# kimkyeonghun/MSA

Hardware: AMD Instinct MI355X
Metric: train-step samples/sec (higher is better)
Workload: dtype bf16; 1 GPU; MMBertForPretraining train step, 3 passes S=50/550/550, 12-layer d=768 heads=12 vocab=30522, T=50 A=500 V=500, dropout on, AdamW; per_gpu_batch=16, global_batch=16, parallelism=dp1, scores_dtype=bf16, mlm_backward=labelled rows only (exact: unlabelled rows have zero CE gradient), deterministic=True

## Files before the change

### msa_amd/csrc/gemm.hip

```cpp
#include "common.h"
#include <atomic>
#include <cstdio>
#include <cstdlib>
#include <cstring>
#include <type_traits>

typedef __attribute__((ext_vector_type(4))) unsigned u32x4;
typedef __attribute__((ext_vector_type(2))) unsigned u32x2;

#define EPI_BIAS 1
#define EPI_GELU 2
#define EPI_RESID 4
#define EPI_GELU_BWD 8
#define EPI_OUT_F32 16

struct GemmNT {
    const bf16_t* A; const bf16_t* B; void* C;
    const float* bias; const bf16_t* R; bf16_t* aux; const bf16_t* U; const float* alpha_dev;
    int M, N, K, lda, ldb, ldc, ldr, ldaux, ldu;
    float alpha;
    uint32_t drop_stream, drop_thr16; float drop_scale;
    int kt_per_split; long long split_stride;
    int* tile_counter; int* tile_counter_next;
    int queue_xcd;
    int group_m;
};

__device__ __forceinline__ int xcd_remap(int bid, int nwg) {
    const int q = nwg >> 3, r = nwg & 7, x = bid & 7, j = bid >> 3;
    return (x < r ? x * (q + 1) : r * (q + 1) + (x - r) * q) + j;
}

__device__ __forceinline__ void ntp_tile_mn(int t, int tiles_m, int tiles_n, int gm, int& tm, int& tn) {
    if (gm <= 1) { tm = t / tiles_n; tn = t - tm * tiles_n; return; }
    const int per = gm * tiles_n, g = t / per, r = t - g * per;
    const int gs = min(gm, tiles_m - g * gm);
    tn = r / gs;
    tm = g * gm + (r - tn * gs);
}

template <int EPI>
__device__ __forceinline__ void epi_store(const GemmNT& p, int m, int n, float (&v)[4]) {
    if constexpr (EPI & EPI_BIAS) {
        const float4 b = *(const float4*)(p.bias + n);
        v[0] += b.x; v[1] += b.y; v[2] += b.z; v[3] += b.w;
    }
    if constexpr (EPI & EPI_GELU) {
        if (p.aux) {
            bf16x4 u = {f2bf(v[0]), f2bf(v[1]), f2bf(v[2]), f2bf(v[3])};
            *(bf16x4*)(p.aux + (size_t)m * p.ldaux + n) = u;
        }
#pragma unroll
        for (int r = 0; r < 4; ++r) v[r] = gelu_erf(v[r]);
    }
    if constexpr (EPI & EPI_GELU_BWD) {
        const bf16x4 u = *(const bf16x4*)(p.U + (size_t)m * p.ldu + n);
#pragma unroll
        for (int r = 0; r < 4; ++r) v[r] *= gelu_erf_grad(bf2f(u[r]));
    }
    if constexpr (EPI & EPI_RESID) {
        if (p.drop_thr16) {
            bool k[4];
            mmb_keep4(p.drop_stream, (uint64_t)m * p.N + n, p.drop_thr16, k);
#pragma unroll
            for (int r = 0; r < 4; ++r) v[r] = k[r] ? v[r] * p.drop_scale : 0.f;
        }
        const bf16x4 rr = *(const bf16x4*)(p.R + (size_t)m * p.ldr + n);
#pragma unroll
        for (int r = 0; r < 4; ++r) v[r] += bf2f(rr[r]);
    }
    if constexpr (EPI & EPI_OUT_F32) {
        *(float4*)((float*)p.C + (size_t)m * p.ldc + n) = make_float4(v[0], v[1], v[2], v[3]);
    } else {
        bf16x4 o = {f2bf(v[0]), f2bf(v[1]), f2bf(v[2]), f2bf(v[3])};
        *(bf16x4*)((bf16_t*)p.C + (size_t)m * p.ldc + n) = o;
    }
}

template <int EPI>
__device__ __forceinline__ void epi_store8(const GemmNT& p, int m, int n, float (&v)[8]) {
    if constexpr (EPI & EPI_BIAS) {
        const float4 b0 = *(const float4*)(p.bias + n), b1 = *(const float4*)(p.bias + n + 4);
        v[0] += b0.x; v[1] += b0.y; v[2] += b0.z; v[3] += b0.w; v[4] += b1.x; v[5] += b1.y; v[6] += b1.z; v[7] += b1.w;
    }
    if constexpr (EPI & EPI_GELU) {
        if (p.aux) {
            bf16x8 u;
#pragma unroll
            for (int r = 0; r < 8; ++r) u[r] = f2bf(v[r]);
            *(bf16x8*)(p.aux + (size_t)m * p.ldaux + n) = u;
        }
#pragma unroll
        for (int r = 0; r < 8; ++r) v[r] = gelu_erf(v[r]);
    }
    if constexpr (EPI & EPI_GELU_BWD) {
        const bf16x8 u = *(const bf16x8*)(p.U + (size_t)m * p.ldu + n);
#pragma unroll
        for (int r = 0; r < 8; ++r) v[r] *= gelu_erf_grad(bf2f(u[r]));
    }
    if constexpr (EPI & EPI_RESID) {
        if (p.drop_thr16) {
            bool k0[4], k1[4];
            const uint64_t idx = (uint64_t)m * p.N + n;
            mmb_keep4(p.drop_stream, idx, p.drop_thr16, k0);
            mmb_keep4(p.drop_stream, idx + 4, p.drop_thr16, k1);
#pragma unroll
            for (int r = 0; r < 4; ++r) { v[r] = k0[r] ? v[r] * p.drop_scale : 0.f; v[4 + r] = k1[r] ? v[4 + r] * p.drop_scale : 0.f; }
        }
        const bf16x8 rr = *(const bf16x8*)(p.R + (size_t)m * p.ldr + n);
#pragma unroll
        for (int r = 0; r < 8; ++r) v[r] += bf2f(rr[r]);
    }
    if constexpr (EPI & EPI_OUT_F32) {
        float* c = (float*)p.C + (size_t)m * p.ldc + n;
        *(float4*)c = make_float4(v[0], v[1], v[2], v[3]);
        *(float4*)(c + 4) = make_float4(v[4], v[5], v[6], v[7]);
    } else {
        bf16x8 o;
#pragma unroll
        for (int r = 0; r < 8; ++r) o[r] = f2bf(v[r]);
        *(bf16x8*)((bf16_t*)p.C + (size_t)m * p.ldc + n) = o;
    }
}

template <int EPI>
__global__ __launch_bounds__(256, 2) void gemm_nt_kernel(const GemmNT p) {
    extern __shared__ __attribute__((aligned(16))) char smem[];
    const int tid = threadIdx.x, lane = tid & 63;
    const int wave = __builtin_amdgcn_readfirstlane(tid >> 6);
    const int wm = wave >> 1, wn = wave & 1;
    const int tiles_n = (p.N + 127) >> 7, tiles_m = (p.M + 127) >> 7;
    const int tile = xcd_remap(blockIdx.x, tiles_m * tiles_n);
    const int m0 = (tile / tiles_n) << 7, n0 = (tile % tiles_n) << 7;
    const int kt0 = p.kt_per_split ? (int)blockIdx.z * p.kt_per_split : 0;
    const int kt1 = p.kt_per_split ? min(p.K >> 6, kt0 + p.kt_per_split) : (p.K >> 6);

    const int srow = lane >> 3, schunk = (lane & 7) ^ srow;
    const bf16_t* a_src[4]; const bf16_t* b_src[4];
#pragma unroll
    for (int i = 0; i < 4; ++i) {
        const int r = (wave * 4 + i) * 8 + srow;
        const int ra = min(m0 + r, p.M - 1), rb = min(n0 + r, p.N - 1);
        a_src[i] = p.A + (size_t)ra * p.lda + schunk * 8;
        b_src[i] = p.B + (size_t)rb * p.ldb + schunk * 8;
    }
    auto stage = [&](int buf, int kt) {
        char* base = smem + buf * 32768 + wave * 4096;
#pragma unroll
        for (int i = 0; i < 4; ++i) {
            __builtin_amdgcn_global_load_lds(GPTR(a_src[i] + kt * 64), LPTR(base + i * 1024), 16, 0, 0);
            __builtin_amdgcn_global_load_lds(GPTR(b_src[i] + kt * 64), LPTR(base + 16384 + i * 1024), 16, 0, 0);
        }
    };

    f32x4 acc[4][4];
#pragma unroll
    for (int i = 0; i < 4; ++i)
#pragma unroll
        for (int j = 0; j < 4; ++j) acc[i][j] = (f32x4){0.f, 0.f, 0.f, 0.f};

    const int fr = lane & 15, fq = lane >> 4;
    auto compute = [&](int buf) {
        const char* As = smem + buf * 32768;
        const char* Bs = As + 16384;
#pragma unroll
        for (int kk = 0; kk < 2; ++kk) {
            bf16x8 af[4], bfr[4];
#pragma unroll
            for (int i = 0; i < 4; ++i) {
                const int ra = wm * 64 + i * 16 + fr, rb = wn * 64 + i * 16 + fr;
                af[i] = *(const bf16x8*)(As + ra * 128 + (((kk * 4 + fq) ^ (ra & 7)) << 4));
                bfr[i] = *(const bf16x8*)(Bs + rb * 128 + (((kk * 4 + fq) ^ (rb & 7)) << 4));
            }
#pragma unroll
            for (int i = 0; i < 4; ++i)
#pragma unroll
                for (int j = 0; j < 4; ++j)
                    acc[i][j] = __builtin_amdgcn_mfma_f32_16x16x32_bf16(bfr[j], af[i], acc[i][j], 0, 0, 0);
        }
    };

    stage(0, kt0);
    asm volatile("s_waitcnt vmcnt(0)" ::: "memory");
    __syncthreads();
    int cur = 0;
    for (int kt = kt0; kt < kt1 - 1; ++kt) {
        stage(cur ^ 1, kt + 1);
        compute(cur);
        asm volatile("s_waitcnt vmcnt(0)" ::: "memory");
        __syncthreads();
        cur ^= 1;
    }
    compute(cur);

    const float alpha = p.alpha * (p.alpha_dev ? *p.alpha_dev : 1.0f);
#pragma unroll
    for (int i = 0; i < 4; ++i) {
        const int m = m0 + wm * 64 + i * 16 + fr;
        if (m >= p.M) continue;
#pragma unroll
        for (int j = 0; j < 4; ++j) {
            const int n = n0 + wn * 64 + j * 16 + fq * 4;
            if (n >= p.N) continue;
            float v[4];
#pragma unroll
            for (int r = 0; r < 4; ++r) v[r] = acc[i][j][r] * alpha;
            if constexpr (EPI == EPI_OUT_F32) {
                if (p.kt_per_split) {
                    *(float4*)((float*)p.C + (size_t)blockIdx.z * p.split_stride + (size_t)m * p.ldc + n) = make_float4(v[0], v[1], v[2], v[3]);
                    continue;
                }
            }
            epi_store<EPI>(p, m, n, v);
        }
    }
}

template <int EPI>
static int launch_nt(hipStream_t s, const GemmNT& p) {
    const int tiles = ((p.M + 127) / 128) * ((p.N + 127) / 128);
    static std::atomic<unsigned long long> attr_done{0};
    if (int e = mmb_allow_lds((const void*)gemm_nt_kernel<EPI>, 65536, attr_done)) return e;
    hipLaunchKernelGGL(gemm_nt_kernel<EPI>, dim3(tiles), dim3(256), 65536, s, p);
    MMB_CHECK_LAUNCH();
    return 0;
}

#ifdef MMB_STAMPS
__device__ unsigned long long* g_stamps = nullptr;
#define MMB_STAMP(var) { __builtin_amdgcn_sched_barrier(0); asm volatile("s_memtime %0\n\ts_waitcnt lgkmcnt(0)" : "=s"(var) :: "memory"); __builtin_amdgcn_sched_barrier(0); }
#else
#define MMB_STAMP(var)
#endif

static std::atomic<int> g_nt_force{0};
static int device_cus() { return mmb_device_cus(); }

__host__ __device__ constexpr int mmb_waitcnt(int vm, int lgkm) { return (vm & 15) | ((vm >> 4) << 14) | 0x70 | (lgkm << 8); }

template <int OFF>
__device__ __forceinline__ void lds_read16f(f32x4& dst, uint32_t lds_addr) {
    asm volatile("ds_read_b128 %0, %1 offset:%2" : "=v"(dst) : "v"(lds_addr), "i"(OFF) : "memory");
}


template <int EPI, bool MULTI, int MQ>
__global__ __launch_bounds__(512, 2) void gemm_nt8_kernel(const GemmNT p) {
#if __HIP_DEVICE_COMPILE__
    extern __shared__ __attribute__((aligned(16))) char smem[];
    const int tid = threadIdx.x, lane = tid & 63;
    const int wave = __builtin_amdgcn_readfirstlane(tid >> 6);
    const int wr = wave >> 2, wc = wave & 3;
    constexpr int MQ0 = (MQ == 7) ? 4 : MQ, MQ1 = (MQ == 7) ? 3 : MQ, NB = MQ0 + MQ1;
    constexpr int BMT = 32 * NB;
    const int tiles_n = (p.N + 255) >> 8, tiles_m = (p.M + BMT - 1) / BMT;
    const int ntiles = tiles_m * tiles_n, G = gridDim.x;
    const int nt = p.K >> 6;
    const float alpha_all = __builtin_bit_cast(float, __builtin_amdgcn_readfirstlane(__builtin_bit_cast(int, p.alpha * (p.alpha_dev ? *p.alpha_dev : 1.0f))));

    const auto rsA = __builtin_amdgcn_make_buffer_rsrc((void*)p.A, 0, (int)((uint32_t)p.M * (uint32_t)p.lda * 2u), 0x00020000);
    const auto rsB = __builtin_amdgcn_make_buffer_rsrc((void*)p.B, 0, (int)((uint32_t)p.N * (uint32_t)p.ldb * 2u), 0x00020000);
    struct Src { uint32_t a[2][2], b[2][2]; };
    auto set_src = [&](int v, Src& o) {
        int l = lane;
        asm volatile("" : "+v"(l));
        int tmi, tni;
        ntp_tile_mn(xcd_remap(v, ntiles), tiles_m, tiles_n, p.group_m, tmi, tni);
        const int tm0 = tmi * BMT, tn0 = tni << 8;
        const int pos = l & 7;
#pragma unroll
        for (int i = 0; i < 2; ++i) {
            const int j = wave + 8 * i, r = 8 * j + (l >> 3);
            const uint32_t chunk_a = (uint32_t)(pos ^ ((r >> 1) & 7));
            const uint32_t chunk_b = (uint32_t)(pos ^ (((r >> 1) & 1) | (((r >> 3) & 3) << 1)));
#pragma unroll
            for (int h = 0; h < 2; ++h) {
                const int mqh = h ? MQ1 : MQ0;
                const int ga = tm0 + (r / (16 * mqh)) * (16 * NB) + (h ? 16 * MQ0 : 0) + (r % (16 * mqh));
                const int gb = tn0 + (r >> 5) * 64 + h * 32 + (r & 31);
                o.a[h][i] = ((uint32_t)min(ga, p.M - 1) * (uint32_t)p.lda + chunk_a * 8u) * 2u;
                o.b[h][i] = ((uint32_t)min(gb, p.N - 1) * (uint32_t)p.ldb + chunk_b * 8u) * 2u;
            }
        }
    };
    Src cur;
    set_src(blockIdx.x, cur);
    Src nxt_store;
    Src& nxt = MULTI ? nxt_store : cur;
    if constexpr (MULTI) nxt_store = cur;
    auto stage_c = [&](auto apw_c, int buf, int which, const Src& o, int kt) {
        constexpr int APW = decltype(apw_c)::value;
        const uint32_t kb = (uint32_t)kt * 128u;
        const int h = which >> 1;
        char* base = smem + buf * 65536 + ((which & 1) ? 0 : 32768) + h * 16384 + wave * 1024;
        if (which & 1) {
            __builtin_amdgcn_raw_ptr_buffer_load_lds(rsA, LPTR(base), 16, o.a[h][0], kb, 0, 0);
            const int mqh = h ? MQ1 : MQ0;
            if (mqh == 4 || (mqh == 3 && APW == 2)) __builtin_amdgcn_raw_ptr_buffer_load_lds(rsA, LPTR(base + 8192), 16, o.a[h][1], kb, 0, 0);
        } else {
            __builtin_amdgcn_raw_ptr_buffer_load_lds(rsB, LPTR(base), 16, o.b[h][0], kb, 0, 0);
            __builtin_amdgcn_raw_ptr_buffer_load_lds(rsB, LPTR(base + 8192), 16, o.b[h][1], kb, 0, 0);
        }
    };

    typedef const __attribute__((address_space(3))) char* lds_cptr;
    typedef const __attribute__((address_space(3))) bf16x8* lds_frag;
    const int fr = lane & 15, fq = lane >> 4;
    const int swa = ((fq ^ (fr >> 1)) & 7) << 4;
    const int swb = ((fq ^ (((fr >> 1) & 1) | ((fr >> 2) << 1))) & 7) << 4;
    const lds_cptr a_rd = (lds_cptr)LPTR(smem) + (wr * (16 * MQ0) + fr) * 128;
    const lds_cptr b_rd = (lds_cptr)LPTR(smem) + 32768 + (wc * 32 + 8 * (fr >> 2) + (fr & 3)) * 128;
    lds_cptr a_rd1 = a_rd + 65536, b_rd1 = b_rd + 65536;
    asm volatile("" : "+v"(a_rd1), "+v"(b_rd1));

    bf16x8 af[2][MQ0], b0f[2][2], b1f[2][2];
    f32x4 acc[NB][4];

    auto read_a = [&](int buf, int h) {
        lds_cptr ab = buf ? a_rd1 : a_rd;
        if (MQ0 != MQ1 && h) ab += wr * (16 * (MQ1 - MQ0) * 128);
#pragma unroll
        for (int ks = 0; ks < 2; ++ks)
#pragma unroll
            for (int i = 0; i < MQ0; ++i)
                if (i < (h ? MQ1 : MQ0)) af[ks][i] = *(lds_frag)(ab + h * 16384 + i * 2048 + (swa ^ (ks * 64)));
    };
    auto read_b = [&](int buf, int h, bf16x8 (&bf)[2][2]) {
        const lds_cptr bb = buf ? b_rd1 : b_rd;
#pragma unroll
        for (int ks = 0; ks < 2; ++ks)
#pragma unroll
            for (int j = 0; j < 2; ++j) bf[ks][j] = *(lds_frag)(bb + h * 16384 + j * 512 + (swb ^ (ks * 64)));
    };
    auto mma = [&](int qa, int qb, const bf16x8 (&bf)[2][2], bool first) {
#pragma unroll
        for (int ks = 0; ks < 2; ++ks)
#pragma unroll
            for (int i = 0; i < MQ0; ++i)
#pragma unroll
                for (int j = 0; j < 2; ++j) {
                    if (i >= (qa ? MQ1 : MQ0)) continue;
                    f32x4& c = acc[qa * MQ0 + i][qb * 2 + j];
                    c = __builtin_amdgcn_mfma_f32_16x16x32_bf16(bf[ks][j], af[ks][i], (first && ks == 0) ? (f32x4){0.f, 0.f, 0.f, 0.f} : c, 0, 0, 0);
                }
    };

    auto body = [&](auto apw_c) {
    constexpr int INFL = 4 + (MQ0 == 4 ? 2 : (MQ0 == 2 ? 1 : decltype(apw_c)::value));
    auto stage = [&](int buf, int which, const Src& o, int kt) { stage_c(apw_c, buf, which, o, kt); };
    const int qx = (MULTI && p.queue_xcd) ? (int)(blockIdx.x & 7) : 0, qs = (MULTI && p.queue_xcd) ? 8 : 1;
    auto queue_fetch = [](int* counter) {
        int r;
        asm volatile("s_nop 4\n\tglobal_atomic_add %0, %1, %2, %3 sc0" : "=&v"(r) : "v"(0), "v"(1), "s"(counter) : "memory");
        return r;
    };
    auto vq_write = [&](int value) {
        const uint32_t vq_addr = (uint32_t)(size_t)LPTR(smem) + 131072u;
        asm volatile("ds_write_b32 %0, %1\n\ts_waitcnt lgkmcnt(0)" :: "v"(vq_addr), "v"(value) : "memory");
    };
    int first_fetch = 0;
    if constexpr (MULTI) { if (p.tile_counter && tid == 0) first_fetch = queue_fetch(p.tile_counter + qx); }
    stage(0, 0, cur, 0); stage(0, 1, cur, 0); stage(0, 2, cur, 0); stage(0, 3, cur, 0);
    stage(1, 0, cur, 1); stage(1, 1, cur, 1); stage(1, 2, cur, 1);
    __builtin_amdgcn_s_waitcnt(mmb_waitcnt(INFL, 15));
    if constexpr (MULTI) {
        if (p.tile_counter && tid == 0) {
            asm volatile("" : "+v"(first_fetch) :: "memory");
            vq_write(G + qs * first_fetch + qx);
        }
    }
    __builtin_amdgcn_s_barrier();
    if (wr == 1) __builtin_amdgcn_s_barrier();

#define NT8_PHASE(READS, LGK_BEFORE_BARRIER, STAGE, VMWAIT, QA, QB, BF, FIRST)                                       \
    {                                                                                                               \
        READS;                                                                                                      \
        STAGE;                                                                                                      \
        if (LGK_BEFORE_BARRIER >= 0) __builtin_amdgcn_s_waitcnt(mmb_waitcnt(63, LGK_BEFORE_BARRIER < 0 ? 0 : LGK_BEFORE_BARRIER)); \
        if (VMWAIT >= 0) __builtin_amdgcn_s_waitcnt(mmb_waitcnt(VMWAIT < 0 ? 0 : VMWAIT, 15));                       \
        __builtin_amdgcn_s_barrier();                                                                               \
        __builtin_amdgcn_s_waitcnt(mmb_waitcnt(63, 0));                                                             \
        __builtin_amdgcn_sched_barrier(0);                                                                          \
        __builtin_amdgcn_s_setprio(1);                                                                              \
        mma(QA, QB, BF, FIRST);                                                                                     \
        __builtin_amdgcn_s_setprio(0);                                                                              \
        __builtin_amdgcn_s_barrier();                                                                               \
        __builtin_amdgcn_sched_barrier(0);                                                                          \
    }
#define NT8_KTILE(D, S1, K1, S2, K2, FIRST)                                                                                   \
    NT8_PHASE((read_b(D, 0, b0f), __builtin_amdgcn_sched_barrier(0), read_a(D, 0)), 2 * MQ0, stage(D ^ 1, 3, S1, K1), -1, 0, 0, b0f, FIRST) \
    NT8_PHASE(read_b(D, 1, b1f), -1, stage(D, 0, S2, K2), -1, 0, 1, b1f, FIRST)                                               \
    NT8_PHASE(read_a(D, 1), -1, stage(D, 1, S2, K2), -1, 1, 1, b1f, FIRST)                                                    \
    NT8_PHASE((void)0, -1, stage(D, 2, S2, K2), INFL, 1, 0, b0f, FIRST)

    for (int v = blockIdx.x, vn = ntiles; v < ntiles; v = vn) {
        int tmi, tni;
// ... 495 lines not shown
                if (accum) { v.x += old[u][jb].x; v.y += old[u][jb].y; v.z += old[u][jb].z; v.w += old[u][jb].w; }
                *(float4*)(out + (size_t)n * K + k) = v;
            }
        }
    }
    if (do_bias) {
        float* red = (float*)smem;
        float v[2][2];
#pragma unroll
        for (int hb = 0; hb < 2; ++hb)
#pragma unroll
            for (int j = 0; j < 2; ++j) {
                float s = bsum[hb][j];
                s += __shfl_xor(s, 16, 64);
                s += __shfl_xor(s, 32, 64);
                v[hb][j] = s;
            }
        __syncthreads();
        if (wr == 1 && fq == 0) {
#pragma unroll
            for (int hb = 0; hb < 2; ++hb)
#pragma unroll
                for (int j = 0; j < 2; ++j) red[((wc * 2 + hb) * 2 + j) * 16 + fr] = v[hb][j];
        }
        __syncthreads();
        if (wr == 0 && fq == 0) {
#pragma unroll
            for (int hb = 0; hb < 2; ++hb)
#pragma unroll
                for (int j = 0; j < 2; ++j) {
                    const int n = n0 + hb * 128 + wc * 32 + j * 16 + fr;
                    if (n >= N) continue;
                    const float bv = (v[hb][j] + red[((wc * 2 + hb) * 2 + j) * 16 + fr]) * alpha;
                    if (split > 0 && gq.bias_slab) gq.bias_slab[(size_t)(split - 1) * gq.bias_stride + bias_off + n] = bv;
                    else atomicAdd(biasp + n, bv);
                }
        }
    }
#ifdef MMB_STAMPS
    if (g_stamps && tid == 0) {
        asm volatile("s_waitcnt vmcnt(0)" ::: "memory");
        asm volatile("s_memrealtime %0\n\ts_waitcnt lgkmcnt(0)" : "=s"(tr1) :: "memory");
        unsigned long long te;
        MMB_STAMP(te)
        unsigned long long* o = g_stamps + ((size_t)(blockIdx.y * gridDim.x + blockIdx.x)) * 6;
        o[0] = ts1 - ts0; o[1] = (unsigned long long)(nt > 0 ? 2 * nt : 0); o[2] = te - ts1; o[3] = 1; o[4] = tr0; o[5] = tr1;
    }
#endif
#endif
}

struct TNReduce { float* W[TN_MAXP]; long long off[TN_MAXP + 1]; int nprob, splits, accumulate; long long slab_stride;
                  float* bias[TN_MAXP]; long long boff[TN_MAXP + 1]; const float* bias_slab; long long bias_stride; };
__global__ void tn_reduce_kernel(const TNReduce r, const float* __restrict__ slab) {
    if (r.bias_slab) {
        const long long nb = r.boff[r.nprob];
        for (long long e = blockIdx.x * (long long)blockDim.x + threadIdx.x; e < nb; e += (long long)gridDim.x * blockDim.x) {
            int lo = 0, hi = r.nprob - 1;
            while (lo < hi) { const int mid = (lo + hi + 1) >> 1; if (r.boff[mid] <= e) lo = mid; else hi = mid - 1; }
            if (!r.bias[lo]) continue;
            float v = r.bias[lo][e - r.boff[lo]];
            for (int s = 0; s + 1 < r.splits; ++s) v += r.bias_slab[(size_t)s * r.bias_stride + e];
            r.bias[lo][e - r.boff[lo]] = v;
        }
    }
    const long long total4 = r.off[r.nprob] >> 2;
    for (long long i = blockIdx.x * (long long)blockDim.x + threadIdx.x; i < total4; i += (long long)gridDim.x * blockDim.x) {
        const long long e = i << 2;
        int lo = 0, hi = r.nprob - 1;
        while (lo < hi) { const int mid = (lo + hi + 1) >> 1; if (r.off[mid] <= e) lo = mid; else hi = mid - 1; }
        float* W = r.W[lo];
        const long long o = r.off[lo];
        float4* dst = (float4*)(W + (e - o));
        float4 v = *dst;
        for (int s = 0; s + 1 < r.splits; ++s) {
            const float4 t = *(const float4*)(slab + (size_t)s * r.slab_stride + e);
            v.x += t.x; v.y += t.y; v.z += t.z; v.w += t.w;
        }
        *dst = v;
    }
}

__global__ __launch_bounds__(256) void colsum_kernel(const bf16_t* __restrict__ X, int M, int N, int ldx, float* __restrict__ out, float alpha, const float* alpha_dev, int rows_per_block) {
    const int lane = threadIdx.x & 63, sub = threadIdx.x >> 6;
    const int n = (blockIdx.x * 64 + lane) * 8;
    const int mbeg = blockIdx.y * rows_per_block, mend = min(M, mbeg + rows_per_block);
    float s[8];
#pragma unroll
    for (int r = 0; r < 8; ++r) s[r] = 0.f;
    if (n < N) {
        int m = mbeg + sub;
        for (; m + 12 < mend; m += 16) {
            bf16x8 v[4];
#pragma unroll
            for (int u = 0; u < 4; ++u) v[u] = *(const bf16x8*)(X + (size_t)(m + 4 * u) * ldx + n);
#pragma unroll
            for (int u = 0; u < 4; ++u)
#pragma unroll
                for (int r = 0; r < 8; ++r) s[r] += bf2f(v[u][r]);
        }
        for (; m < mend; m += 4) {
            const bf16x8 v = *(const bf16x8*)(X + (size_t)m * ldx + n);
#pragma unroll
            for (int r = 0; r < 8; ++r) s[r] += bf2f(v[r]);
        }
    }
    __shared__ float red[4][64][9];
#pragma unroll
    for (int r = 0; r < 8; ++r) red[sub][lane][r] = s[r];
    __syncthreads();
    if (sub == 0 && n < N) {
        const float a = alpha * (alpha_dev ? *alpha_dev : 1.0f);
#pragma unroll
        for (int r = 0; r < 8; ++r)
            atomicAdd(out + n + r, (red[0][lane][r] + red[1][lane][r] + red[2][lane][r] + red[3][lane][r]) * a);
    }
}

extern "C" {

__global__ void nt_splitk_reduce_kernel(const float* __restrict__ slabs, int splits, long long stride, int M, int N, bf16_t* __restrict__ C, int ldc,
                                        const bf16_t* __restrict__ R, int ldr) {
    const long long i = ((long long)blockIdx.x * blockDim.x + threadIdx.x) * 4;
    if (i >= (long long)M * N) return;
    float4 a = *(const float4*)(slabs + i);
    for (int z = 1; z < splits; ++z) { const float4 b = *(const float4*)(slabs + z * stride + i); a.x += b.x; a.y += b.y; a.z += b.z; a.w += b.w; }
    const int m = (int)(i / N), n = (int)(i - (long long)m * N);
    if (R) { const bf16x4 r = *(const bf16x4*)(R + (size_t)m * ldr + n); a.x += bf2f(r[0]); a.y += bf2f(r[1]); a.z += bf2f(r[2]); a.w += bf2f(r[3]); }
    bf16x4 o = {f2bf(a.x), f2bf(a.y), f2bf(a.z), f2bf(a.w)};
    *(bf16x4*)(C + (size_t)m * ldc + n) = o;
}

static int nt_splitk_plan(int M, int N, int K) {
    const int tiles = ((M + 127) / 128) * ((N + 127) / 128), kt = K >> 6;
    int splits = (2 * device_cus() + tiles - 1) / tiles;
    if (splits > kt / 4) splits = kt / 4;
    if (splits < 1) splits = 1;
    return splits;
}
size_t mmbert_gemm_nt_splitk_workspace(int M, int N, int K) { return (size_t)nt_splitk_plan(M, N, K) * M * N * sizeof(float); }

int mmbert_gemm_nt_splitk(hipStream_t stream, const void* A, int lda, const void* B, int ldb, void* C, int ldc,
                          int M, int N, int K, void* workspace, const void* R, int ldr) {
    if (M <= 0 || N <= 0) return 0;
    if (K <= 0 || (K & 63) || (N & 3) || (lda & 7) || (ldb & 7) || (ldc & 3) || !workspace || (R && (ldr & 3))) return -1;
    GemmNT p = {};
    p.A = (const bf16_t*)A; p.B = (const bf16_t*)B; p.C = workspace; p.M = M; p.N = N; p.K = K; p.lda = lda; p.ldb = ldb; p.ldc = N;
    p.alpha = 1.0f;
    const int splits = nt_splitk_plan(M, N, K), kt = K >> 6;
    p.kt_per_split = (kt + splits - 1) / splits;
    p.split_stride = (long long)M * N;
    const int zs = (kt + p.kt_per_split - 1) / p.kt_per_split;
    static std::atomic<unsigned long long> attr_done{0};
    if (int e = mmb_allow_lds((const void*)gemm_nt_kernel<EPI_OUT_F32>, 65536, attr_done)) return e;
    hipLaunchKernelGGL(gemm_nt_kernel<EPI_OUT_F32>, dim3(((M + 127) / 128) * ((N + 127) / 128), 1, zs), dim3(256), 65536, stream, p);
    MMB_CHECK_LAUNCH();
    const long long n4 = ((long long)M * N + 3) / 4;
    hipLaunchKernelGGL(nt_splitk_reduce_kernel, dim3((unsigned)((n4 + 255) / 256)), dim3(256), 0, stream, (const float*)workspace, zs, p.split_stride, M, N, (bf16_t*)C, ldc,
                       (const bf16_t*)R, ldr);
    MMB_CHECK_LAUNCH();
    return 0;
}

int mmbert_gemm_nt(hipStream_t stream, const void* A, int lda, const void* B, int ldb, void* C, int ldc,
                   int M, int N, int K, int epi, const float* bias, const void* R, int ldr, void* aux, int ldaux,
                   const void* U, int ldu, float alpha, const float* alpha_dev,
                   uint32_t drop_stream, uint32_t drop_thr16, float drop_scale, int* tile_queue) {
    if (M <= 0 || N <= 0) return 0;
    if (K <= 0 || (K & 63) || (N & 3) || (lda & 7) || (ldb & 7) || (ldc & 3)) return -1;
    GemmNT p;
    p.A = (const bf16_t*)A; p.B = (const bf16_t*)B; p.C = C; p.bias = bias; p.R = (const bf16_t*)R;
    p.aux = (bf16_t*)aux; p.U = (const bf16_t*)U; p.alpha_dev = alpha_dev;
    p.M = M; p.N = N; p.K = K; p.lda = lda; p.ldb = ldb; p.ldc = ldc; p.ldr = ldr; p.ldaux = ldaux; p.ldu = ldu;
    p.alpha = alpha; p.drop_stream = drop_stream; p.drop_thr16 = drop_thr16; p.drop_scale = drop_scale;
    p.kt_per_split = 0; p.split_stride = 0; p.group_m = 1;
    p.tile_counter = tile_queue; p.tile_counter_next = tile_queue ? tile_queue + 8 : nullptr;
    switch (epi) {
        case 0: return dispatch_nt<0>(stream, p);
        case EPI_BIAS: return dispatch_nt<EPI_BIAS>(stream, p);
        case EPI_BIAS | EPI_GELU: return dispatch_nt<EPI_BIAS | EPI_GELU>(stream, p);
        case EPI_BIAS | EPI_RESID: return dispatch_nt<EPI_BIAS | EPI_RESID>(stream, p);
        case EPI_RESID: return dispatch_nt<EPI_RESID>(stream, p);
        case EPI_GELU_BWD: return dispatch_nt<EPI_GELU_BWD>(stream, p);
        case EPI_OUT_F32: return dispatch_nt<EPI_OUT_F32>(stream, p);
        case EPI_BIAS | EPI_OUT_F32: return dispatch_nt<EPI_BIAS | EPI_OUT_F32>(stream, p);
        default: return -2;
    }
}

int mmbert_gemm_nt_describe(int M, int N, int K, int epi, int with_queue, int* out) {
    if (!out || M <= 0 || N <= 0 || K <= 0) return -1;
    GemmNT p = {};
    p.M = M; p.N = N; p.K = K; p.lda = K; p.ldb = K; p.ldc = N; p.ldr = (epi & (EPI_RESID)) ? N : 0; p.ldaux = (epi & EPI_GELU) ? N : 0;
    p.ldu = (epi & EPI_GELU_BWD) ? N : 0;
    static int dummy_queue[16];
    p.tile_counter = with_queue ? dummy_queue : nullptr;
    const NTChoice c = nt_choose(p, epi);
    const int cus = device_cus();
    out[0] = c.kernel; out[1] = c.bm; out[2] = c.kernel == NTK_128 ? 128 : 256; out[3] = c.tiles; out[4] = c.workgroups;
    out[5] = (int)(100.0 * c.tiles / cus + 0.5); out[6] = c.group_m; out[7] = cus;
    return 0;
}

#ifdef MMB_STAMPS
int mmbert_debug_set_stamps(void* buf) {
    return (int)hipMemcpyToSymbol(HIP_SYMBOL(g_stamps), &buf, sizeof(buf));
}
#endif
void mmbert_gemm_nt_force(int mode) {
    g_nt_force.store((mode == 1 || mode == 8 || mode == 128 || mode == 192 || mode == 224 || mode == 256) ? mode : 0);
}

static std::atomic<int> g_tn_splits{0};
void mmbert_gemm_tn_force_splits(int splits) { g_tn_splits.store(splits); }
static std::atomic<int> g_tn_one_launch{0};
void mmbert_gemm_tn_force_one_launch(int on) { g_tn_one_launch.store(on ? 1 : 0); }
static int tn_plan(int nprob, const int* N, const int* K, int M, int* splits_out, int* tiles_out) {
    int tiles = 0;
    double elems = 0;
    for (int i = 0; i < nprob; ++i) { tiles += ((N[i] + 255) / 256) * ((K[i] + 255) / 256); elems += (double)N[i] * K[i]; }
    constexpr double T_ROW = 21e-9, T_FIX = 8e-6;
    const int slots = device_cus();
    const int max_splits = (M + 511) / 512;
    double cost[9];
    double best_cost = 1e300;
    int top = 1;
    for (int sp = 1; sp <= 8 && sp <= (max_splits < 1 ? 1 : max_splits); ++sp) {
        const long long wgs = (long long)tiles * sp;
        const long long rounds = (wgs + slots - 1) / slots;
        const double rows = (double)((M + sp - 1) / sp);
        cost[sp] = (rows * T_ROW + T_FIX) * (double)rounds + (sp - 1) * elems * 8.0 / 9.4e12;
        if (cost[sp] < best_cost) best_cost = cost[sp];
        top = sp;
    }
    int best = 1;
    for (int sp = 1; sp <= top; ++sp)
        if (cost[sp] <= 1.03 * best_cost) { best = sp; break; }
    int splits = best;
    if (tiles >= slots && nprob > 8) splits = 1;
    if (g_tn_splits.load() > 0) splits = g_tn_splits.load();
    if (splits > max_splits) splits = max_splits;
    if (splits < 1) splits = 1;
    *splits_out = splits; *tiles_out = tiles;
    return 0;
}

size_t mmbert_gemm_tn_grouped_workspace(int nprob, const int* N, const int* K, int M, int* splits_out) {
    int splits, tiles;
    tn_plan(nprob, N, K, M, &splits, &tiles);
    if (splits_out) *splits_out = splits;
    if (splits == 1) return 0;
    size_t elems = 0, cols = 0;
    for (int i = 0; i < nprob; ++i) { elems += (size_t)N[i] * K[i]; cols += (size_t)N[i]; }
    return (size_t)(splits - 1) * (elems + cols) * sizeof(float);
}

size_t mmbert_gemm_tn_workspace(int M, int N, int K, int* splits_out) {
    return mmbert_gemm_tn_grouped_workspace(1, &N, &K, M, splits_out);
}

int mmbert_gemm_tn_grouped_rows(hipStream_t stream, int nprob, const void* const* A, const int* lda, const void* const* B, const int* ldb,
                                float* const* W, float* const* bias, const int* N, const int* K, const int* Mrows,
                                int accumulate, const int* accumulate_each, float alpha, const float* alpha_dev, void* slab) {
    if (nprob <= 0) return 0;
    if (nprob > TN_MAXP) return -1;
    const int M = Mrows[0];
    if (M <= 0) return 0;
    int nlong = 0;
    while (nlong < nprob && Mrows[nlong] == M) ++nlong;
    for (int i = nlong; i < nprob; ++i)
        if (Mrows[i] >= M || Mrows[i] <= 0) return -1;
    GemmTNG g;
    int splits, tiles_long, tiles_all;
    tn_plan(nlong, N, K, M, &splits, &tiles_long);
    if (nlong < nprob) splits = 1;
    long long off = 0, boff = 0;
    int tile0 = 0;
    TNReduce r;
    for (int i = 0; i < nprob; ++i) {
        if ((N[i] & 7) || (K[i] & 7) || (lda[i] & 7) || (ldb[i] & 7) || N[i] < 8 || K[i] < 8) return -1;
        TNProb& q = g.pr[i];
        q.A = (const bf16_t*)A[i]; q.B = (const bf16_t*)B[i]; q.W = W[i]; q.bias = bias ? bias[i] : nullptr;
        q.N = N[i]; q.K = K[i]; q.lda = lda[i]; q.ldb = ldb[i]; q.M = Mrows[i]; q.acc = accumulate_each ? accumulate_each[i] : accumulate;
        q.tiles_k = (K[i] + 255) / 256; q.tile0 = tile0; q.slab_off = (int)off; q.bias_off = (int)boff;
        r.W[i] = W[i]; r.off[i] = off; r.bias[i] = q.bias; r.boff[i] = boff;
        boff += N[i];
        tile0 += ((N[i] + 255) / 256) * q.tiles_k;
        off += (long long)N[i] * K[i];
    }
    tiles_all = tile0;
    if (splits > 1 && off > 0x7fffffffLL) return -1;
    for (int i = nprob; i < TN_MAXP; ++i) { g.pr[i] = g.pr[0]; g.pr[i].tile0 = 0x7fffffff; r.W[i] = nullptr; r.bias[i] = nullptr; }
    for (int i = nprob; i <= TN_MAXP; ++i) { r.off[i] = off; r.boff[i] = boff; }
    if (splits > 1 && !slab) return -3;
    g.slab = (float*)slab; g.alpha_dev = alpha_dev; g.slab_stride = off;
    const bool det_bias = splits > 1 && mmb_deterministic();
    g.bias_slab = det_bias ? (float*)slab + (size_t)(splits - 1) * off : nullptr;
    g.bias_stride = boff;
    r.bias_slab = g.bias_slab; r.bias_stride = boff; g.nprob = nprob; g.total_tiles = tiles_all; g.M = M;
    g.splits = splits; g.rows_per_split = (((M + splits - 1) / splits) + 31) / 32 * 32; g.accumulate = accumulate; g.alpha = alpha;
    static std::atomic<unsigned long long> attr_done8{0};
    if (int e = mmb_allow_lds((const void*)gemm_tn8_kernel, 131072, attr_done8)) return e;
    auto kern = gemm_tn8_kernel;
    const int cus_ = device_cus();
    const int tiles_short = tiles_all - tiles_long;
    if (splits == 1 && (tiles_long > cus_ || tiles_short > 0)) {
        const int step_ = g_tn_one_launch.load() ? (tiles_long > 0 ? tiles_long : 1) : cus_;
        for (int base = 0; base < tiles_long; base += step_) {
// ... 52 lines not shown
```

Before: 1262 samples/s.

## Deepen NT GEMM LDS pipeline to multi-stage with counted waits and flattened split-K grid

Turns the 128x128 NT GEMM kernel's double-buffered loop into an NS-stage ring of LDS buffers using counted vmcnt waits and a single barrier per k-step. LDS fragments are read with inline ds_read_b128 and split lgkm waits, so the second k-half's reads can overlap the first half's MFMAs. Grids with at most one tile per CU use 4 stages (128KB LDS), and others keep 2. The split-K path folds z into a flattened, XCD-remapped 1D grid. The deeper stages lower occupancy to one block per CU, and the attribute call for the 2-stage path is skipped, so that path relies on the default LDS limit.

```diff
diff --git a/msa_amd/csrc/gemm.hip b/msa_amd/csrc/gemm.hip
--- a/msa_amd/csrc/gemm.hip
+++ b/msa_amd/csrc/gemm.hip
@@ -123,17 +123,34 @@
     }
 }
 
-template <int EPI>
+__host__ __device__ constexpr int mmb_waitcnt(int vm, int lgkm) { return (vm & 15) | ((vm >> 4) << 14) | 0x70 | (lgkm << 8); }
+
+template <int OFF>
+__device__ __forceinline__ void lds_read16f(f32x4& dst, uint32_t lds_addr) {
+    asm volatile("ds_read_b128 %0, %1 offset:%2" : "=v"(dst) : "v"(lds_addr), "i"(OFF) : "memory");
+}
+
+template <int EPI, int NS>
 __global__ __launch_bounds__(256, 2) void gemm_nt_kernel(const GemmNT p) {
     extern __shared__ __attribute__((aligned(16))) char smem[];
+    static_assert(NS >= 2 && NS <= 4, "the drain's counted waits are written out for up to 4 stages");
     const int tid = threadIdx.x, lane = tid & 63;
     const int wave = __builtin_amdgcn_readfirstlane(tid >> 6);
     const int wm = wave >> 1, wn = wave & 1;
     const int tiles_n = (p.N + 127) >> 7, tiles_m = (p.M + 127) >> 7;
-    const int tile = xcd_remap(blockIdx.x, tiles_m * tiles_n);
+    const int tiles = tiles_m * tiles_n;
+    int tile, z = 0;
+    if (p.kt_per_split) {
+        const int u = xcd_remap(blockIdx.x, gridDim.x);
+        z = u / tiles; tile = u - z * tiles;
+    } else {
+        tile = xcd_remap(blockIdx.x, tiles);
+    }
     const int m0 = (tile / tiles_n) << 7, n0 = (tile % tiles_n) << 7;
-    const int kt0 = p.kt_per_split ? (int)blockIdx.z * p.kt_per_split : 0;
+    const int kt0 = p.kt_per_split ? z * p.kt_per_split : 0;
     const int kt1 = p.kt_per_split ? min(p.K >> 6, kt0 + p.kt_per_split) : (p.K >> 6);
+    const int nk = kt1 - kt0;
+    const float alpha = p.alpha * (p.alpha_dev ? *p.alpha_dev : 1.0f);
 
     const int srow = lane >> 3, schunk = (lane & 7) ^ srow;
     const bf16_t* a_src[4]; const bf16_t* b_src[4];
@@ -141,15 +158,15 @@
     for (int i = 0; i < 4; ++i) {
         const int r = (wave * 4 + i) * 8 + srow;
         const int ra = min(m0 + r, p.M - 1), rb = min(n0 + r, p.N - 1);
-        a_src[i] = p.A + (size_t)ra * p.lda + schunk * 8;
-        b_src[i] = p.B + (size_t)rb * p.ldb + schunk * 8;
-    }
-    auto stage = [&](int buf, int kt) {
-        char* base = smem + buf * 32768 + wave * 4096;
+        a_src[i] = p.A + (size_t)ra * p.lda + schunk * 8 + (size_t)kt0 * 64;
+        b_src[i] = p.B + (size_t)rb * p.ldb + schunk * 8 + (size_t)kt0 * 64;
+    }
+    auto stage = [&](int slot, int t) {
+        char* base = smem + slot * 32768 + wave * 4096;
 #pragma unroll
         for (int i = 0; i < 4; ++i) {
-            __builtin_amdgcn_global_load_lds(GPTR(a_src[i] + kt * 64), LPTR(base + i * 1024), 16, 0, 0);
-            __builtin_amdgcn_global_load_lds(GPTR(b_src[i] + kt * 64), LPTR(base + 16384 + i * 1024), 16, 0, 0);
+            __builtin_amdgcn_global_load_lds(GPTR(a_src[i] + t * 64), LPTR(base + i * 1024), 16, 0, 0);
+            __builtin_amdgcn_global_load_lds(GPTR(b_src[i] + t * 64), LPTR(base + 16384 + i * 1024), 16, 0, 0);
         }
     };
 
@@ -160,40 +177,58 @@
         for (int j = 0; j < 4; ++j) acc[i][j] = (f32x4){0.f, 0.f, 0.f, 0.f};
 
     const int fr = lane & 15, fq = lane >> 4;
-    auto compute = [&](int buf) {
-        const char* As = smem + buf * 32768;
-        const char* Bs = As + 16384;
+    const uint32_t lds0 = (uint32_t)(size_t)LPTR(smem);
+    const uint32_t a_rd = lds0 + (uint32_t)((wm * 64 + fr) * 128), b_rd = lds0 + 16384u + (uint32_t)((wn * 64 + fr) * 128);
+    const uint32_t sw0 = (uint32_t)((fq ^ (fr & 7)) << 4), sw1 = (uint32_t)(((4 + fq) ^ (fr & 7)) << 4);
+    auto compute = [&](int slot) {
+        const uint32_t so = (uint32_t)slot * 32768u;
+        f32x4 af[2][4], bfr[2][4];
 #pragma unroll
         for (int kk = 0; kk < 2; ++kk) {
-            bf16x8 af[4], bfr[4];
-#pragma unroll
-            for (int i = 0; i < 4; ++i) {
-                const int ra = wm * 64 + i * 16 + fr, rb = wn * 64 + i * 16 + fr;
-                af[i] = *(const bf16x8*)(As + ra * 128 + (((kk * 4 + fq) ^ (ra & 7)) << 4));
-                bfr[i] = *(const bf16x8*)(Bs + rb * 128 + (((kk * 4 + fq) ^ (rb & 7)) << 4));
-            }
+            const uint32_t aa = a_rd + so + (kk ? sw1 : sw0), bb = b_rd + so + (kk ? sw1 : sw0);
+            lds_read16f<0>(af[kk][0], aa); lds_read16f<2048>(af[kk][1], aa); lds_read16f<4096>(af[kk][2], aa); lds_read16f<6144>(af[kk][3], aa);
+            lds_read16f<0>(bfr[kk][0], bb); lds_read16f<2048>(bfr[kk][1], bb); lds_read16f<4096>(bfr[kk][2], bb); lds_read16f<6144>(bfr[kk][3], bb);
+        }
+#pragma unroll
+        for (int kk = 0; kk < 2; ++kk) {
+            if (kk == 0)
+                asm volatile("s_waitcnt lgkmcnt(8)" : "+v"(af[0][0]), "+v"(af[0][1]), "+v"(af[0][2]), "+v"(af[0][3]),
+                             "+v"(bfr[0][0]), "+v"(bfr[0][1]), "+v"(bfr[0][2]), "+v"(bfr[0][3]) :: "memory");
+            else
+                asm volatile("s_waitcnt lgkmcnt(0)" : "+v"(af[1][0]), "+v"(af[1][1]), "+v"(af[1][2]), "+v"(af[1][3]),
+                             "+v"(bfr[1][0]), "+v"(bfr[1][1]), "+v"(bfr[1][2]), "+v"(bfr[1][3]) :: "memory");
 #pragma unroll
             for (int i = 0; i < 4; ++i)
 #pragma unroll
                 for (int j = 0; j < 4; ++j)
-                    acc[i][j] = __builtin_amdgcn_mfma_f32_16x16x32_bf16(bfr[j], af[i], acc[i][j], 0, 0, 0);
-        }
-    };
-
-    stage(0, kt0);
-    asm volatile("s_waitcnt vmcnt(0)" ::: "memory");
-    __syncthreads();
-    int cur = 0;
-    for (int kt = kt0; kt < kt1 - 1; ++kt) {
-        stage(cur ^ 1, kt + 1);
-        compute(cur);
-        asm volatile("s_waitcnt vmcnt(0)" ::: "memory");
-        __syncthreads();
-        cur ^= 1;
-    }
-    compute(cur);
-
-    const float alpha = p.alpha * (p.alpha_dev ? *p.alpha_dev : 1.0f);
+                    acc[i][j] = __builtin_amdgcn_mfma_f32_16x16x32_bf16(__builtin_bit_cast(bf16x8, bfr[kk][j]), __builtin_bit_cast(bf16x8, af[kk][i]), acc[i][j], 0, 0, 0);
+        }
+    };
+
+#pragma unroll
+    for (int s = 0; s < NS - 1; ++s)
+        if (s < nk) stage(s, s);
+    int i = 0, slot = 0;
+    for (; i + NS - 1 < nk; ++i) {
+        asm volatile("s_waitcnt vmcnt(%0)" :: "n"(8 * (NS - 2)) : "memory");
+        __builtin_amdgcn_s_barrier();
+        stage(slot == 0 ? NS - 1 : slot - 1, i + NS - 1);
+        compute(slot);
+        slot = slot == NS - 1 ? 0 : slot + 1;
+    }
+#pragma unroll
+    for (int r = NS - 2; r >= 0; --r) {
+        if (i + r == nk - 1) {
+            if (r == 2) asm volatile("s_waitcnt vmcnt(16)" ::: "memory");
+            else if (r == 1) asm volatile("s_waitcnt vmcnt(8)" ::: "memory");
+            else asm volatile("s_waitcnt vmcnt(0)" ::: "memory");
+            __builtin_amdgcn_s_barrier();
+            compute(slot);
+            slot = slot == NS - 1 ? 0 : slot + 1;
+            ++i;
+        }
+    }
+
 #pragma unroll
     for (int i = 0; i < 4; ++i) {
         const int m = m0 + wm * 64 + i * 16 + fr;
@@ -207,7 +242,7 @@
             for (int r = 0; r < 4; ++r) v[r] = acc[i][j][r] * alpha;
             if constexpr (EPI == EPI_OUT_F32) {
                 if (p.kt_per_split) {
-                    *(float4*)((float*)p.C + (size_t)blockIdx.z * p.split_stride + (size_t)m * p.ldc + n) = make_float4(v[0], v[1], v[2], v[3]);
+                    *(float4*)((float*)p.C + (size_t)z * p.split_stride + (size_t)m * p.ldc + n) = make_float4(v[0], v[1], v[2], v[3]);
                     continue;
                 }
             }
@@ -216,12 +251,20 @@
     }
 }
 
+#define NT_DEEP_STAGES 4
+#define NT_MANY_STAGES 2
+#define NT_SPLITK_STAGES 4
+static int device_cus();
 template <int EPI>
 static int launch_nt(hipStream_t s, const GemmNT& p) {
     const int tiles = ((p.M + 127) / 128) * ((p.N + 127) / 128);
     static std::atomic<unsigned long long> attr_done{0};
-    if (int e = mmb_allow_lds((const void*)gemm_nt_kernel<EPI>, 65536, attr_done)) return e;
-    hipLaunchKernelGGL(gemm_nt_kernel<EPI>, dim3(tiles), dim3(256), 65536, s, p);
+    if (tiles <= device_cus()) {
+        if (int e = mmb_allow_lds((const void*)gemm_nt_kernel<EPI, NT_DEEP_STAGES>, NT_DEEP_STAGES * 32768, attr_done)) return e;
+        hipLaunchKernelGGL((gemm_nt_kernel<EPI, NT_DEEP_STAGES>), dim3(tiles), dim3(256), NT_DEEP_STAGES * 32768, s, p);
+    } else {
+        hipLaunchKernelGGL((gemm_nt_kernel<EPI, NT_MANY_STAGES>), dim3(tiles), dim3(256), NT_MANY_STAGES * 32768, s, p);
+    }
     MMB_CHECK_LAUNCH();
     return 0;
 }
@@ -235,13 +278,6 @@
 
 static std::atomic<int> g_nt_force{0};
 static int device_cus() { return mmb_device_cus(); }
-
-__host__ __device__ constexpr int mmb_waitcnt(int vm, int lgkm) { return (vm & 15) | ((vm >> 4) << 14) | 0x70 | (lgkm << 8); }
-
-template <int OFF>
-__device__ __forceinline__ void lds_read16f(f32x4& dst, uint32_t lds_addr) {
-    asm volatile("ds_read_b128 %0, %1 offset:%2" : "=v"(dst) : "v"(lds_addr), "i"(OFF) : "memory");
-}
 
 
 template <int EPI, bool MULTI, int MQ>
@@ -1043,8 +1079,8 @@
     p.split_stride = (long long)M * N;
     const int zs = (kt + p.kt_per_split - 1) / p.kt_per_split;
     static std::atomic<unsigned long long> attr_done{0};
-    if (int e = mmb_allow_lds((const void*)gemm_nt_kernel<EPI_OUT_F32>, 65536, attr_done)) return e;
-    hipLaunchKernelGGL(gemm_nt_kernel<EPI_OUT_F32>, dim3(((M + 127) / 128) * ((N + 127) / 128), 1, zs), dim3(256), 65536, stream, p);
+    if (int e = mmb_allow_lds((const void*)gemm_nt_kernel<EPI_OUT_F32, NT_SPLITK_STAGES>, NT_SPLITK_STAGES * 32768, attr_done)) return e;
+    hipLaunchKernelGGL((gemm_nt_kernel<EPI_OUT_F32, NT_SPLITK_STAGES>), dim3(((M + 127) / 128) * ((N + 127) / 128) * zs), dim3(256), NT_SPLITK_STAGES * 32768, stream, p);
     MMB_CHECK_LAUNCH();
     const long long n4 = ((long long)M * N + 3) / 4;
     hipLaunchKernelGGL(nt_splitk_reduce_kernel, dim3((unsigned)((n4 + 255) / 256)), dim3(256), 0, stream, (const float*)workspace, zs, p.split_stride, M, N, (bf16_t*)C, ldc,
```

Result: no change. 1268 samples/s, median of 6 (+0.5%).
